# ValerioSpagnoli/Monocular-Visual-Inertial-MSCKF

Measured on AMD Instinct MI355X. Metric: MSCKF measurement-updates/sec (N=30 clones, 2000 features, track=10), higher is better.
Workload: dtype f64; 1 GPU; N=30 clones, F=2000 features, track=10, fp64; unit_definition=one 2000-feature measurement update (K1-K7)

## Files before the change

monocular-visual-inertial-msckf_amd/csrc/k_feature.h:

```cpp
#pragma once
#include <hip/hip_runtime.h>
#include "wave_ops.h"
#include "feature_dpp_groups.h"
#include "batch_order.h"

namespace msckf {


struct FeatureArgs {
    int F;
    int f0;
    int ldp;
    const int* view_ptr;
    const double* obs_uv;
    const int* obs_slot;
    const double* obs_w;
    const double* idp_base;
    const double* idp_m;
    const double* idp_rho;
    const double* cam_R;
    const double* cam_t;
    const double* cam_R0;
    const double* cam_t0;
    const double* P;
    const double* chi2;
    int n_chi2;
    double g[3];
    double Kinv[9];
    double sigma2;
    const long long* blk_off;
    void* stack;
    int stack_f32;
    int* rank;
    unsigned char* accepted;
    const unsigned char* select;
    double* gamma;
    long long* stamps;
    long long zero_idx;
    const SplitRec* split;
    int* rank_h;
    unsigned char* acc_h;
};

__host__ __device__ inline int feature_chunk_views(int M) {
    const int a = (6 * M + 63) / 64, b = (M + 9) / 10;
    const int nch = a > b ? a : b;
    return (M + nch - 1) / nch;
}
__host__ __device__ inline int feature_lds_doubles(int M, bool chunked) {
    const int R2 = 2 * M, C6 = 6 * M;
    const int head = (M + 2) / 2 + R2 * 6 + R2 * 3 + 3 * C6;
    if (!chunked) {
        const int stage = R2 * (6 * feature_chunk_views(M) + 1), elim = (R2 + 1) * (R2 + 3);
        return head + (stage > elim ? stage : elim) + 3 * R2 + 8;
    }
    const int stage = R2 * (6 * feature_chunk_views(M) + 1) + (R2 + 2), elim = (R2 + 1) * (R2 + 3);
    return head + (stage > elim ? stage : elim) + 8;
}

__host__ __device__ inline int feature_split_estride(int M) {
    const int R2 = 2 * M;
    const int cv = feature_chunk_views(M), ld = 6 * (cv > SPLIT_GSLOTS ? cv : SPLIT_GSLOTS) + 1;
    const int stage = R2 * ld, elim = (R2 + 1) * (R2 + 3);
    return (stage > elim ? stage : elim) + 8;
}
__host__ __device__ inline int feature_split_lds_doubles(int M, int nwv = 1) {
    const int R2 = 2 * M, C6 = 6 * M;
    const int head = (M + 2) / 2 + R2 * 6 + R2 * 3 + 3 * C6;
    const int cv = feature_chunk_views(M), ld = 6 * (cv > SPLIT_GSLOTS ? cv : SPLIT_GSLOTS) + 1;
    const int tail = (R2 + 2) + 8 + 6 * R2 + 6 * C6 + (M + 3 * SPLIT_MAXG + 4) / 2 + 2;
    if (nwv > 1) return head + nwv * feature_split_estride(M) + tail;
    return head + R2 * ld + tail;
}

// ... 57 lines not shown
                 : "+v"(d[0]), "+v"(d[1]), "+v"(d[2]), "+v"(d[3]) : "v"(a[0]), "v"(a[1]), "v"(a[2]), "v"(a[3]), [w] "v"(w), [lk] "i"(LK));
}
#undef MSCKF_FD
template <int LK, int J0, int NJ>
__device__ __forceinline__ void elim_from16(double (&d)[16], const double (&a)[16], double w) {
    if constexpr (NJ > 0) {
        constexpr int N1 = NJ < 4 ? NJ : 4;
        double dd[N1], aa[N1];
#pragma unroll
        for (int i = 0; i < N1; ++i) { dd[i] = d[J0 + i]; aa[i] = a[J0 + i]; }
        elim_from<LK>(dd, aa, w);
#pragma unroll
        for (int i = 0; i < N1; ++i) d[J0 + i] = dd[i];
        elim_from16<LK, J0 + N1, NJ - N1>(d, a, w);
    }
}
template <int LK, int J0, int NJ>
__device__ __forceinline__ void elim_self16(double (&d)[16], double w) {
    if constexpr (NJ > 0) {
        constexpr int N1 = NJ < 4 ? NJ : 4;
        double dd[N1];
#pragma unroll
        for (int i = 0; i < N1; ++i) dd[i] = d[J0 + i];
        elim_self<LK>(dd, w);
#pragma unroll
        for (int i = 0; i < N1; ++i) d[J0 + i] = dd[i];
        elim_self16<LK, J0 + N1, NJ - N1>(d, w);
    }
}
template <int K, int KEND, typename Fn>
__device__ __forceinline__ void feature_static_for(Fn&& fn) {
    if constexpr (K < KEND) { fn(FTag<K>{}); feature_static_for<K + 1, KEND>(fn); }
}
template <int RMAX, bool SPLIT = false, int NWV = 1>
__global__ __launch_bounds__(64 * NWV, NWV > 1 ? 1 : (RMAX <= 24 ? 3 : 2)) void k_feature(FeatureArgs p) {
    constexpr bool CHUNKED = RMAX > 32;
    static_assert(!SPLIT || CHUNKED, "the split form is an instance of the chunked kernel");
    static_assert(NWV == 1 || SPLIT, "several wavefronts per track: the split form only");
    constexpr bool ONE_CHUNK = RMAX <= 24;
    constexpr int MAXVK = ONE_CHUNK ? 10 : (RMAX - 2) / 2;
    extern __shared__ __attribute__((aligned(16))) double smem[];
    const int f = blockIdx.x + p.f0;
    const int lane = threadIdx.x & 63, wv = NWV > 1 ? (int)(threadIdx.x >> 6) : 0;
    const bool wfirst = wv == 0;
    auto xsync = [&]() { if constexpr (NWV > 1) __syncthreads(); else wave_sync(); };
    const int v0 = p.view_ptr[f];
    const int M = p.view_ptr[f + 1] - v0;
    const int R2 = 2 * M, C6 = 6 * M;
    int* sSlot = reinterpret_cast<int*>(smem);
    double* sA = smem + (M + 2) / 2;
    double* sV = sA + R2 * 6;
    double* sZ = sV + R2 * 3;

    if (f == 0 && lane < 8 && wfirst) {
        if (p.stack_f32) static_cast<float*>(p.stack)[p.zero_idx + lane] = 0.0f;
        else static_cast<double*>(p.stack)[p.zero_idx + lane] = 0.0;
    }
    auto wsum = [&](double x) -> double {
        if constexpr (RMAX <= 34) {
            x = row16_sum(x);
            return readlane_d(x, 0) + readlane_d(x, 16);
        } else {
            return wave_sum(x);
        }
    };
    if (p.select && !(p.select[f] & 1)) {
        if (lane == 0 && wfirst) {
            p.rank[f] = 0; p.gamma[f] = 0.0; p.accepted[f] = 3;
            if (p.acc_h) { p.rank_h[f] = 0; p.acc_h[f] = 3; }
            if constexpr (SPLIT) {
                const SplitRec& sr = p.split[blockIdx.x];
                for (int g = 0; g < sr.ng; ++g) if (sr.child[g] >= 0) { p.rank[sr.child[g]] = 3; p.accepted[sr.child[g]] = 3; }
                p.rank[sr.wide] = 0; p.accepted[sr.wide] = 3;
            }
        }
        return;
    }
    long long tq[8] = {0, 0, 0, 0, 0, 0, 0, 0};
    if (p.stamps) tq[0] = wall_clock64();
    double res = 0.0, a0 = 0, a1 = 0, a2 = 0, a3 = 0, a4 = 0, a5 = 0, h0 = 0, h1 = 0, h2 = 0;
    const int view = lane >> 1;
    if (lane < R2) {
        const int o = v0 + view;
        const int s = p.obs_slot[o];
        if ((lane & 1) == 0 && wfirst) sSlot[view] = s;
        const double* R = p.cam_R + 9 * s;
        const double* t = p.cam_t + 3 * s;
        const double* R0 = p.cam_R0 + 9 * s;
        const double* t0 = p.cam_t0 + 3 * s;
        const double rho = p.idp_rho[f];
        const double wx = rho * (p.idp_base[3 * f + 0] - t[0]) + p.idp_m[3 * f + 0];
        const double wy = rho * (p.idp_base[3 * f + 1] - t[1]) + p.idp_m[3 * f + 1];
        const double wz = rho * (p.idp_base[3 * f + 2] - t[2]) + p.idp_m[3 * f + 2];
        const double px = R[0] * wx + R[3] * wy + R[6] * wz;
        const double py = R[1] * wx + R[4] * wy + R[7] * wz;
        const double pz = R[2] * wx + R[5] * wy + R[8] * wz;
        const double Wx = R[0] * px + R[1] * py + R[2] * pz + t[0];
        const double Wy = R[3] * px + R[4] * py + R[5] * pz + t[1];
        const double Wz = R[6] * px + R[7] * py + R[8] * pz + t[2];
        const double u = p.obs_uv[2 * o], v = p.obs_uv[2 * o + 1];
        double wv = 1.0;
        if (p.obs_w) wv = p.obs_w[o];
        const double zx = p.Kinv[0] * u + p.Kinv[1] * v + p.Kinv[2];
        const double zy = p.Kinv[3] * u + p.Kinv[4] * v + p.Kinv[5];
        const double zw = p.Kinv[6] * u + p.Kinv[7] * v + p.Kinv[8];
        const double ia = 1.0 / pz;
        const double jb = -px * (ia * ia);
        const double jc = -py * (ia * ia);
        const double izw = 1.0 / zw;
        const double gx = p.g[0], gy = p.g[1], gz = p.g[2];
        const double u0 = R0[0] * gx + R0[3] * gy + R0[6] * gz;
        const double u1 = R0[1] * gx + R0[4] * gy + R0[7] * gz;
        const double u2 = R0[2] * gx + R0[5] * gy + R0[8] * gz;
        const double ex = Wx - t0[0], ey = Wy - t0[1], ez = Wz - t0[2];
        const double u3 = ey * gz - ez * gy;
        const double u4 = ez * gx - ex * gz;
        const double u5 = ex * gy - ey * gx;
        const double den = u0 * u0 + u1 * u1 + u2 * u2 + u3 * u3 + u4 * u4 + u5 * u5;
        double J0, J1, J2;
        if ((lane & 1) == 0) {
            res = zx * izw - px * ia;
            J0 = ia; J1 = 0.0; J2 = jb;
            a0 = -jb * py; a1 = -ia * pz + jb * px; a2 = ia * py;
        } else {
            res = zy * izw - py * ia;
            J0 = 0.0; J1 = ia; J2 = jc;
            a0 = ia * pz - jc * py; a1 = jc * px; a2 = -ia * px;
        }
        h0 = J0 * R[0] + J1 * R[1] + J2 * R[2];
        h1 = J0 * R[3] + J1 * R[4] + J2 * R[5];
        h2 = J0 * R[6] + J1 * R[7] + J2 * R[8];
        a3 = -h0; a4 = -h1; a5 = -h2;
        if (den > 1e-6) {
// ... 148 lines not shown
                for (int a = 0; a < 6; ++a) pb[VW % (PD + 1)][a] = prow[(size_t)a * p.ldp];
            }
        };
        fetch(FTag<0>{});
        if constexpr (PD > 1) fetch(FTag<1>{});
        if constexpr (PD > 2) fetch(FTag<2>{});
        if constexpr (PD > 3) fetch(FTag<3>{});
        static_assert(PD >= 1 && PD <= 4, "the prologue above issues PD views");
        {
            const double z0 = sZ[c], z1 = sZ[C6 + c], z2 = sZ[2 * C6 + c];
            const double d0 = sA[(2 * vwc) * 6 + ac], d1 = sA[(2 * vwc + 1) * 6 + ac];
            auto rows = [&](auto tagl) {
                constexpr int L0 = decltype(tagl)::value;
                if (L0 < R2) {
                    double x[4] = {0.0, 0.0, 0.0, 0.0};
                    corr(tagl, x, z0, z1, z2);
#pragma unroll
                    for (int i = 0; i < 4; ++i)
                        if (L0 + i < R2 && cok) sE[(L0 + i) * ldE + lc] = x[i];
                }
            };
            rows(FTag<0>{}); rows(FTag<4>{}); rows(FTag<8>{}); rows(FTag<12>{}); rows(FTag<16>{}); rows(FTag<20>{});
            rows(FTag<24>{}); rows(FTag<28>{});
            if (cok) {
                sE[(2 * vwc) * ldE + lc] += d0;
                sE[(2 * vwc + 1) * ldE + lc] += d1;
            }
            if (last && lane < R2) sE[lane * ldE + cw] = ro;
            wave_sync();
            const int nel = q * cwp;
            if (cw == C6) {
                const double* srcrows = sE + rank * ldE;
                if (p.stack_f32) {
                    float* blk = static_cast<float*>(p.stack) + p.blk_off[f];
                    for (int e = lane; e < nel; e += 64) blk[e] = (float)srcrows[e];
                } else {
                    double* blk = static_cast<double*>(p.stack) + p.blk_off[f];
                    int e = lane;
                    for (; e + 192 < nel; e += 256) {
                        const double x0 = srcrows[e], x1 = srcrows[e + 64], x2 = srcrows[e + 128], x3 = srcrows[e + 192];
                        blk[e] = x0; blk[e + 64] = x1; blk[e + 128] = x2; blk[e + 192] = x3;
                    }
                    for (; e < nel; e += 64) blk[e] = srcrows[e];
                }
            } else {
                const float inv_cwp = 1.0f / (float)cwp;
                for (int e = lane; e < nel; e += 64) {
                    const int L = (int)(((float)e + 0.5f) * inv_cwp), cc = e - L * cwp;
                    const double x = sE[(rank + L) * ldE + cc];
                    const long long dst = p.blk_off[f] + (long long)L * ldb + c0 + cc;
                    if (p.stack_f32) static_cast<float*>(p.stack)[dst] = (float)x;
                    else static_cast<double*>(p.stack)[dst] = x;
                }
            }
            wave_sync();
        }
        if (p.stamps && vc0 == 0) tq[3] = wall_clock64();
        {
            double zp0 = 0, zp1 = 0, zp2 = 0;
            auto view = [&](auto tagv) {
                constexpr int VW = decltype(tagv)::value;
                if (VW < M) {
                    fetch(FTag<VW + PD>{});
                    double e0 = 0.0, e1 = 0.0;
                    if constexpr (VW < MAXVK) FeatGateView<VW>::run(zp0, zp1, zp2, e0, e1, pb[VW % (PD + 1)], zq, aq);
                    if (cok) { sE[(2 * VW) * ldE + lc] = e0; sE[(2 * VW + 1) * ldE + lc] = e1; }
                }
            };
            view(FTag<0>{}); view(FTag<1>{}); view(FTag<2>{}); view(FTag<3>{}); view(FTag<4>{}); view(FTag<5>{});
            view(FTag<6>{}); view(FTag<7>{}); view(FTag<8>{}); view(FTag<9>{}); view(FTag<10>{});
            view(FTag<11>{}); view(FTag<12>{}); view(FTag<13>{}); view(FTag<14>{});
            auto rows = [&](auto tagl) {
                constexpr int L0 = decltype(tagl)::value;
                if (L0 < R2) {
                    double x[4];
#pragma unroll
                    for (int i = 0; i < 4; ++i) x[i] = sE[min(L0 + i, R2 - 1) * ldE + lc];
                    corr(tagl, x, zp0, zp1, zp2);
#pragma unroll
                    for (int i = 0; i < 4; ++i)
                        if (L0 + i < R2 && cok) sE[(L0 + i) * ldE + lc] = x[i];
                }
            };
// ... 657 lines not shown
```

monocular-visual-inertial-msckf_amd/csrc/msckf_abi.hip:

```cpp
#include <hip/hip_runtime.h>
#include <dlfcn.h>
#include <rccl/rccl.h>

#include <algorithm>
#include <atomic>
#include <chrono>
#include <condition_variable>
#include <functional>
#include <mutex>
#include <thread>
#include <unordered_map>
#include <unordered_set>
#include <pthread.h>
#include <sched.h>
#include <cmath>
#include <cstdio>
#include <cstdlib>
#include <cstring>
#include <string>
#include <vector>

#include "../../include/msckf_mi355x.h"
#include "k_feature.h"
#include "k_fold.h"
// ... 295 lines not shown
    std::vector<double> x_key;
    int x_nrec = 0;
    bool x_plan_valid = false;
    std::vector<SweepNode> x_snodes;
    std::vector<SweepFold> x_sfolds;
    int x_n_merges = 0;
    size_t x_root_off = 0, x_zero_off = 0;
    long long x_rec_base = 0;
    size_t rbuf_doubles = 0;
    size_t gather_off = 0;
    int gather_cap = 0;
    int n_leaves = 0;
    int n_leaves0 = 0;
    float us_host_prep = 0, us_h2d = 0, us_d2h = 0;
    float us_stage[3] = {0, 0, 0};
    float us_total = 0;
    std::vector<int> h_view_in;
    bool have_tracks = false, use_select = false;
    msckf_select_params sel_params{};
    std::vector<double> h_cam[4];
    bool have_nominal = false;
    Buf dNom;
    Buf dPoseArena, dFeatArena, dRawArena, dResArena, dGateArena;
    void *hPose = nullptr, *hFeat = nullptr, *hRes = nullptr, *hGate = nullptr, *hP = nullptr;
    size_t hFeatCap = 0, hGateCap = 0, res_dx_off = 0, res_p_off = 0;
    size_t res_mask_off = 0, res_mask_cap = 0, res_cap = 0;
    std::vector<int> x_bounds;
    int xmask_doubles = 0;
    Buf dPerm;
    bool have_w = false;
    size_t w_raw_off = 0;
    Buf dObsW;
    const GatherRec* gather_rec = nullptr;
    std::vector<double> chi2_cache;
    bool defer_state_sync = false;
    bool oneshot = false;
    bool feature_launched = false;
    HostPool* pool = nullptr;
    Buf dGsEx, dGsFlag, dGsProg;
    Buf dRootFlush, dXRootFlush;
    RootTables plan_tabs, merge_tabs;
    unsigned gs_epoch = 0;
    bool gs_enabled = true;
    bool gs_overlap = true;
    int root_band = 0;
    bool gs_stamp = false;
    Buf dSplit, dRem;
    static constexpr int REM_DIRECT_DEFAULT = 3840;
    int rem_leaf_rows = 0;
    int rem_direct_max = REM_DIRECT_DEFAULT, rem_direct_max_wide = 16 * GS_MAX_NB2;
    bool retry_plain = false;
    bool fake_timeout_done = false;
    bool rem_direct = false;
    std::vector<FoldNode> rnodes;
    std::vector<std::pair<int, int>> rlevels;
    int rroot = -1; size_t rroot_off = 0;
    std::vector<int> rtops;
    int rtop_rows = 0;
    int rem_cut_rows = -1;
    Buf dRNodes;
    hipEvent_t ev_rem = nullptr;
    bool wide_active = false;
    bool no_wide = false;
    hipStream_t stream2 = nullptr;
    hipEvent_t ev_fork = nullptr, ev_wfeat = nullptr;
    bool wide_on_stream2 = false;
// ... 769 lines not shown
    if (c->xchg_planned)
        HIPCHK(c, hipMemcpyAsync(c->dRbuf.p, c->h_xflags.data(), c->h_xflags.size() * 8, hipMemcpyHostToDevice, ps));
    HIPCHK(c, hipEventRecord(c->ev_plan_up[img], ps));
    c->plan_staged[img] = true;
    return MSCKF_OK;
}

inline bool rem_in_record(const msckf_ctx* c) { return c->xchg_planned && c->xsplit_rows > 0; }
inline double* rem_rows(msckf_ctx* c) { return rem_in_record(c) ? ptr<double>(c->dRbuf) + rec_rem_off(c) + 1 : ptr<double>(c->dRem); }
inline int* drem_count(msckf_ctx* c) { return reinterpret_cast<int*>(ptr<double>(c->dRem) + (size_t)16 * GS_MAX_NB2 * (6 * c->maxN + 1)); }
inline int* rem_count(msckf_ctx* c) { return rem_in_record(c) ? reinterpret_cast<int*>(ptr<double>(c->dRbuf) + rec_rem_off(c)) : drem_count(c); }

int launch_feature(msckf_ctx* c) {
    if (c->F == 0) return MSCKF_OK;
    FeatureArgs a{};
    a.F = c->F; a.ldp = c->d;
    a.view_ptr = ptr<int>(c->dViewPtr); a.obs_uv = ptr<double>(c->dObsUV); a.obs_slot = ptr<int>(c->dObsSlot);
    a.idp_base = ptr<double>(c->dBase); a.idp_m = ptr<double>(c->dMvec); a.idp_rho = ptr<double>(c->dRho);
    a.obs_w = c->have_w ? ptr<double>(c->dObsW) : nullptr;
    a.cam_R = ptr<double>(c->dCamR); a.cam_t = ptr<double>(c->dCamT);
    a.cam_R0 = ptr<double>(c->dCamR0); a.cam_t0 = ptr<double>(c->dCamT0);
    a.P = ptr<double>(c->dP); a.chi2 = ptr<double>(c->dChi2); a.n_chi2 = c->n_chi2;
    for (int i = 0; i < 3; ++i) a.g[i] = c->g[i];
    for (int i = 0; i < 9; ++i) a.Kinv[i] = c->Kinv[i];
    a.sigma2 = c->sigma * c->sigma;
    a.blk_off = ptr<long long>(c->dBlkOff); a.stack = c->dStack.p; a.stack_f32 = c->cfg.dtype == MSCKF_DTYPE_F32 ? 1 : 0;
    a.rank = ptr<int>(c->dRank); a.accepted = ptr<unsigned char>(c->dAcc); a.gamma = ptr<double>(c->dGamma);
    a.select = c->use_select ? ptr<unsigned char>(c->dSelFlags) : nullptr;
    a.stamps = c->dStamps.p ? ptr<long long>(c->dStamps) + 8 * 8192 : nullptr;
    a.zero_idx = c->ord.stack_elems;
    c->gate_direct = c->want_direct && !c->use_select;
    if (c->gate_direct) { a.rank_h = static_cast<int*>(c->hGate); a.acc_h = static_cast<unsigned char*>(c->hGate) + (size_t)c->ord.Fs * 4; }
    hipStream_t st = c->stream;
    auto go = [&](int f0, int nf, int mmax) {
        if (nf <= 0) return;
        a.f0 = f0; a.F = nf; a.split = nullptr;
        const bool chunked = 2 * mmax + 1 > 32;
        int lds_d = 0;
        for (int m = 1; m <= mmax; ++m) lds_d = std::max(lds_d, feature_lds_doubles(m, chunked));
        const size_t lds = (size_t)lds_d * 8;
        if (mmax <= 10) hipLaunchKernelGGL(k_feature<24>, dim3(nf), dim3(64), lds, st, a);
        else if (2 * mmax + 1 <= 32) hipLaunchKernelGGL(k_feature<32>, dim3(nf), dim3(64), lds, st, a);
        else hipLaunchKernelGGL(k_feature<64>, dim3(nf), dim3(64), lds, st, a);
    };
    auto go_split = [&](int f0, int nf, int mmax) {
        if (nf <= 0) return;
        a.f0 = f0; a.F = nf; a.split = ptr<SplitRec>(c->dSplit);
        static const int mw_max = [] { const char* e = std::getenv("MSCKF_SPLIT_MW_MAX"); return e ? std::atoi(e) : 512; }();
        const int nwv = nf <= mw_max ? 4 : 1;
        int lds_d = 0;
        for (int m = 2; m <= mmax; ++m) lds_d = std::max(lds_d, feature_split_lds_doubles(m, nwv));
        if (nwv == 4) hipLaunchKernelGGL((k_feature<64, true, 4>), dim3(nf), dim3(256), (size_t)lds_d * 8, st, a);
        else hipLaunchKernelGGL((k_feature<64, true>), dim3(nf), dim3(64), (size_t)lds_d * 8, st, a);
        if (c->rem_direct) {
            RemScatterArgs r{};
            r.split = ptr<SplitRec>(c->dSplit); r.n_tracks = nf; r.rows_cap = c->ord.rem_cap;
            r.dc = c->dc; r.N = c->N;
            r.view_ptr = a.view_ptr; r.obs_slot = a.obs_slot; r.blk_off = a.blk_off; r.stack = a.stack; r.stack_f32 = a.stack_f32;
            r.rank = a.rank; r.accepted = a.accepted; r.out = rem_rows(c); r.nrows = rem_count(c);
            hipLaunchKernelGGL(k_rem_scatter, dim3(nf + 1), dim3(256), 0, st, r);
        }
    };
    c->wide_on_stream2 = false;
    if (c->ord.split_on && c->ord.Fw > 0) {
        if (c->wide_concurrent) {
            HIPCHK(c, hipEventRecord(c->ev_fork, c->stream));
            HIPCHK(c, hipStreamWaitEvent(c->stream2, c->ev_fork, 0));
            st = c->stream2;
            go_split(c->ord.Fb, c->ord.Fw, c->ord.Mmax_wide);
            HIPCHK(c, hipEventRecord(c->ev_wfeat, c->stream2));
            c->wide_on_stream2 = true;
            st = c->stream;
            go(0, c->ord.Fb, c->ord.Mmax_band);
        } else {
// ... 653 lines not shown
    c->maxN = cfg->max_clones; c->maxF = cfg->max_features; c->maxM = std::min<int>(cfg->max_track, MSCKF_MAX_TRACK); c->maxV = cfg->max_track;
    if (hipSetDevice(c->device) != hipSuccess) { delete c; return MSCKF_ERR_NO_DEVICE; }
    hipDeviceProp_t prop{};
    if (hipGetDeviceProperties(&prop, c->device) != hipSuccess) { delete c; return MSCKF_ERR_NO_DEVICE; }
    if (std::strncmp(prop.gcnArchName, "gfx950", 6) != 0) { delete c; return MSCKF_ERR_NO_DEVICE; }
    c->n_cu = prop.multiProcessorCount;
    if (hipStreamCreateWithFlags(&c->stream, hipStreamNonBlocking) != hipSuccess) { delete c; return MSCKF_ERR_HIP; }
    if (hipStreamCreateWithFlags(&c->stream2, hipStreamNonBlocking) != hipSuccess) { msckf_destroy(c); return MSCKF_ERR_HIP; }
    if (hipStreamCreateWithFlags(&c->stream_up, hipStreamNonBlocking) != hipSuccess) { msckf_destroy(c); return MSCKF_ERR_HIP; }
    {
        const char* e1 = std::getenv("MSCKF_GAIN_STREAM");
        const char* e2 = std::getenv("MSCKF_GAIN_OVERLAP");
        c->gs_enabled = !(e1 && std::atoi(e1) == 0);
        { const char* e3 = std::getenv("MSCKF_WIDE_STREAM"); c->wide_concurrent = !(e3 && std::atoi(e3) == 0); }
        c->gs_overlap = !(e2 && std::atoi(e2) == 0);
        { const char* e4 = std::getenv("MSCKF_REM_LEAF_ROWS"); if (e4 && std::atoi(e4) >= 16) c->rem_leaf_rows = std::atoi(e4); }
        { const char* e5 = std::getenv("MSCKF_REM_CUT_ROWS"); if (e5 && std::atoi(e5) >= 0) c->rem_cut_rows = std::atoi(e5); }
    }
    hipError_t cerr = hipSuccess;
    const char* cwhat = "";
    auto CK = [&](hipError_t e, const char* what) { if (cerr == hipSuccess && e != hipSuccess) { cerr = e; cwhat = what; } };
    for (auto& e : c->ev) CK(hipEventCreate(&e), "hipEventCreate");
    CK(hipEventCreateWithFlags(&c->ev_fork, hipEventDisableTiming), "hipEventCreate");
    CK(hipEventCreateWithFlags(&c->ev_wfeat, hipEventDisableTiming), "hipEventCreate");
    CK(hipEventCreateWithFlags(&c->ev_rem, hipEventDisableTiming), "hipEventCreate");
    for (auto& e : c->ev_plan_up) CK(hipEventCreateWithFlags(&e, hipEventDisableTiming), "hipEventCreate");
    CK(hipEventCreateWithFlags(&c->ev_state, hipEventDisableTiming), "hipEventCreate");
    CK(hipEventCreateWithFlags(&c->ev_gate, hipEventDisableTiming), "hipEventCreate");
    if (const char* e = std::getenv("MSCKF_DIRECT_RESULT")) c->direct_enabled = std::atoi(e) != 0;
    if (const char* e = std::getenv("MSCKF_ROOT_STREAM")) c->stream_enabled = std::atoi(e) != 0;
    if (const char* e = std::getenv("MSCKF_LEAF_STREAM")) c->leaf_stream_enabled = std::atoi(e) != 0;
    if (const char* e = std::getenv("MSCKF_DEBUG_POISON")) c->ws_poison = std::atoi(e) != 0;
    if (const char* e = std::getenv("MSCKF_PLAN_MEMO")) c->plan_memo = std::atoi(e) != 0;
    auto lds_attr = [&](const void* f, int bytes, const char* what) {
        CK(hipFuncSetAttribute(f, hipFuncAttributeMaxDynamicSharedMemorySize, bytes), what);
    };
    {
#define FK(RPT, CPT) reinterpret_cast<const void*>(&k_fold<FOLD_T, FOLD_RL, RPT, CPT>)
        const void* fk[] = {FK(FOLD_RPT_LEAF, FOLD_CPT1), FK(FOLD_RPT_BIG, FOLD_CPT1), FK(FOLD_RPT_LEAF, FOLD_CPT2),
                            FK(FOLD_RPT_BIG, FOLD_CPT2), FK(FOLD_RPT_W3, FOLD_CPT3)};
#undef FK
        for (const void* f : fk) lds_attr(f, FOLD_LDS_BYTES, "k_fold LDS attribute");
    }
    lds_attr(reinterpret_cast<const void*>(&k_fold_g<FOLDG_T, 12, 6>), FOLD_LDS_BYTES, "k_fold_g LDS attribute");
    lds_attr(reinterpret_cast<const void*>(&k_fold_g<FOLDG_T, 6, 10>), FOLD_LDS_BYTES, "k_fold_g LDS attribute");
    lds_attr(reinterpret_cast<const void*>(&k_fold_g<FOLDG_T, 2, 21>), FOLD_LDS_BYTES, "k_fold_g LDS attribute");
    lds_attr(reinterpret_cast<const void*>(&k_fold_g<FOLDG_T, 1, 42>), FOLD_LDS_BYTES, "k_fold_g LDS attribute");
    {
#define SK(NR, UN) reinterpret_cast<const void*>(&k_solve_lds<NR, SOLVE_WAVES, SOLVE_ROWS, UN>)
        const void* sk[] = {SK(1, true), SK(2, true), SK(3, true), SK(1, false), SK(2, false), SK(3, false)};
#undef SK
        for (const void* f : sk) lds_attr(f, LDS_MAX_BYTES - 1024, "k_solve_lds LDS attribute");
#define SM(NR, MD) reinterpret_cast<const void*>(&k_solve_lds<NR, SOLVE_WAVES, 1, true, MD>)
        const void* sm[] = {SM(1, 1), SM(2, 1), SM(3, 1), SM(1, 2), SM(2, 2), SM(3, 2), SM(1, 3), SM(2, 3), SM(3, 3)};
#undef SM
        for (const void* f : sm) lds_attr(f, LDS_MAX_BYTES - 1024, "k_solve_lds (one-sided) LDS attribute");
    }
    lds_attr(reinterpret_cast<const void*>(&k_sweep<SWEEP_NW, SWEEP_WPF>), FOLD_LDS_BYTES, "k_sweep LDS attribute");
    lds_attr(reinterpret_cast<const void*>(&k_sweep<SWEEP_NW_BIG, 1>), FOLD_LDS_BYTES, "k_sweep<12> LDS attribute");
    lds_attr(reinterpret_cast<const void*>(&k_root_gain<SWEEP_NW, 2>), LDS_MAX_BYTES - 1024, "k_root_gain LDS attribute");
    lds_attr(reinterpret_cast<const void*>(&k_root_gain_m<SWEEP_NW, SWEEP_NW_MID, 2>), LDS_MAX_BYTES - 1024, "k_root_gain_m LDS attribute");
    lds_attr(reinterpret_cast<const void*>(&k_leaf_root_gain<SWEEP_NW, 2>), LDS_MAX_BYTES - 1024, "k_leaf_root_gain LDS attribute");
    lds_attr(reinterpret_cast<const void*>(&k_root_gain_w<SWEEP_NW, 4, 2>), LDS_MAX_BYTES - 1024, "k_root_gain_w LDS attribute");
    lds_attr(reinterpret_cast<const void*>(&k_root_gain_w<SWEEP_NW, 4, 3>), LDS_MAX_BYTES - 1024, "k_root_gain_w LDS attribute");
    lds_attr(reinterpret_cast<const void*>(&k_root_gain_w<SWEEP_NW, 6, 2>), LDS_MAX_BYTES - 1024, "k_root_gain_w LDS attribute");
    lds_attr(reinterpret_cast<const void*>(&k_root_gain_w<SWEEP_NW, 6, 3>), LDS_MAX_BYTES - 1024, "k_root_gain_w LDS attribute");
    lds_attr(reinterpret_cast<const void*>(&k_feature<64, true, 4>), LDS_MAX_BYTES - 1024, "k_feature<64, true, 4> LDS attribute");
    lds_attr(reinterpret_cast<const void*>(&k_gain_stream<1>), LDS_MAX_BYTES - 1024, "k_gain_stream<1> LDS attribute");
    lds_attr(reinterpret_cast<const void*>(&k_gain_stream<2>), LDS_MAX_BYTES - 1024, "k_gain_stream<2> LDS attribute");
    lds_attr(reinterpret_cast<const void*>(&k_gain_dense), LDS_MAX_BYTES - 1024, "k_gain_dense LDS attribute");
    lds_attr(reinterpret_cast<const void*>(&k_lsweep<8, 4, LS_RS4, true>), FOLD_LDS_BYTES, "k_lsweep<8,4> LDS attribute");
    lds_attr(reinterpret_cast<const void*>(&k_lsweep<12, 4, LS_RS4, false>), FOLD_LDS_BYTES, "k_lsweep<12,4> LDS attribute");
    lds_attr(reinterpret_cast<const void*>(&k_lsweep<SWEEP_NW, 6, LS_RS6>), FOLD_LDS_BYTES, "k_lsweep<6> LDS attribute");
    lds_attr(reinterpret_cast<const void*>(&k_lsweep<12, 6, LS_RS6, false>), FOLD_LDS_BYTES, "k_lsweep<12,6> LDS attribute");
    lds_attr(reinterpret_cast<const void*>(&k_lsweep<8, 6, LS_RS6T>), FOLD_LDS_BYTES, "k_lsweep<8,6,tall> LDS attribute");
    lds_attr(reinterpret_cast<const void*>(&k_wsweep<SWEEP_NW, 4>), FOLD_LDS_BYTES, "k_wsweep<4> LDS attribute");
    lds_attr(reinterpret_cast<const void*>(&k_wsweep<SWEEP_NW, 6>), FOLD_LDS_BYTES, "k_wsweep<6> LDS attribute");
    lds_attr(reinterpret_cast<const void*>(&k_chol<512>), LDS_MAX_BYTES - 1024, "k_chol LDS attribute");
    lds_attr(reinterpret_cast<const void*>(&k_feature<24>), LDS_MAX_BYTES - 1024, "k_feature LDS attribute");
    lds_attr(reinterpret_cast<const void*>(&k_feature<32>), LDS_MAX_BYTES - 1024, "k_feature LDS attribute");
    lds_attr(reinterpret_cast<const void*>(&k_feature<64>), LDS_MAX_BYTES - 1024, "k_feature LDS attribute");
    if (((size_t)15 * (15 + 6 * c->maxN) + 225) * 8 > (size_t)(LDS_MAX_BYTES - 1024)) { msckf_destroy(c); return MSCKF_ERR_ARG; }
    lds_attr(reinterpret_cast<const void*>(&k_propagate), LDS_MAX_BYTES - 1024, "k_propagate LDS attribute");
    if (cerr != hipSuccess) {
        std::fprintf(stderr, "msckf_create: %s: %s\n", cwhat, hipGetErrorString(cerr));
        msckf_destroy(c);
        return MSCKF_ERR_HIP;
    }
    const int N = c->maxN, d = 15 + 6 * N, dc = 6 * N;
    int rc = MSCKF_OK;
    auto E = [&](Buf& b, size_t bytes, bool z = false) { if (rc == MSCKF_OK) rc = ensure(c, b, bytes, z); };
    E(c->dP, (size_t)d * d * 8);
    E(c->dPoseArena, (size_t)24 * N * 8);
    c->res_mask_cap = ((size_t)std::max(c->maxF, 1) + 7) & ~(size_t)7;
    c->res_cap = 64 + (size_t)d * 8 + (size_t)d * d * 8 + c->res_mask_cap;
    E(c->dResArena, c->res_cap, true);
    E(c->dGateArena, (size_t)5 * std::max(c->maxF, 1));
    if (rc == MSCKF_OK) {
        set_view(c->dCamR, c->dPoseArena.p, 0, (size_t)N * 72);
        set_view(c->dCamT, c->dPoseArena.p, (size_t)9 * N * 8, (size_t)N * 24);
        set_view(c->dCamR0, c->dPoseArena.p, (size_t)12 * N * 8, (size_t)N * 72);
        set_view(c->dCamT0, c->dPoseArena.p, (size_t)21 * N * 8, (size_t)N * 24);
        c->d = 15;
        seat_result_views(c);
        bool ok = hipHostMalloc(&c->hPose, (size_t)24 * N * 8) == hipSuccess &&
                  hipHostMalloc(&c->hRes, c->res_cap) == hipSuccess &&
                  hipHostMalloc(&c->hGate, (c->hGateCap = (size_t)5 * std::max(c->maxF, 1))) == hipSuccess &&
                  hipHostMalloc(&c->hP, (size_t)d * d * 8) == hipSuccess;
        if (!ok) rc = MSCKF_ERR_HIP;
    }
    E(c->dChi2, 1024 * 8);
    E(c->dKeep, (size_t)d * 4);
    E(c->dY, (size_t)d * dc * 8); E(c->dS, (size_t)dc * dc * 8); E(c->dL, (size_t)dc * dc * 8);
// ... 124 lines not shown
    tracks_clear(c);
    return MSCKF_OK;
}

static int launch_gather_w(msckf_ctx* c) {
    const int Fs = c->ord.Fs;
    char* draw = static_cast<char*>(c->dRawArena.p);
    HIPCHK(c, hipMemcpyAsync(draw + c->w_raw_off, static_cast<char*>(c->hFeat) + c->w_raw_off, (size_t)c->sumM * 8, hipMemcpyHostToDevice, c->stream));
    hipLaunchKernelGGL(k_gather_w, dim3((Fs + GATHER_THREADS / 32 - 1) / (GATHER_THREADS / 32)), dim3(GATHER_THREADS), 0, c->stream,
                       c->gather_rec, reinterpret_cast<const double*>(draw + c->w_raw_off), ptr<double>(c->dObsW), Fs, c->sumM, c->ord.sumMs);
    HIPCHK(c, hipGetLastError());
    return MSCKF_OK;
}

static int set_features_impl(msckf_ctx* c, int32_t F, const int32_t* view_ptr, const double* obs_uv,
                             const int32_t* obs_slot, const double* idp_base, const double* idp_m,
                             const double* idp_rho, const TrackEmitSrc* emit, const double* sigma_view = nullptr) {
    if (!c || F < 0 || F > c->maxF) return MSCKF_ERR_ARG;
    if (!c->have_state) return MSCKF_ERR_STATE;
    if (F > 0 && (!view_ptr || !obs_slot || (!emit && (!obs_uv || !idp_base || !idp_m || !idp_rho)))) return MSCKF_ERR_ARG;
    HIPCHK(c, hipSetDevice(c->device));
    const double t0 = now_us();
    const int N = c->N;
    if (c->feat_busy) { HIPCHK(c, hipStreamSynchronize(c->stream)); c->feat_busy = false; }
    c->have_features = false;
    c->feature_launched = false;
    c->last.ran = false;
    c->have_tracks = false;
    c->use_select = false;
    c->batch_from_store = false;
    c->no_wide = false;
    c->have_w = false;
    c->gather_rec = nullptr;
    if (F == 0) {
        c->F = 0;
        c->sumM = 0; c->ord.reset(); c->nodes.clear(); c->levels.clear(); c->snodes.clear(); c->sfolds.clear(); c->sweep_levels.clear(); c->n_group_merges = 0;
        c->band_plan = false; c->root = -1;
        c->wide_active = false;
        c->rem_direct = false;
        c->rnodes.clear(); c->rlevels.clear(); c->rroot = -1; c->rtops.clear(); c->rtop_rows = 0;
        c->plan_valid = false;
        c->xchg_planned = false;
        if (c->xchg) {
            const size_t need = (rec_head(c) + (size_t)N * rec_slot(c) + rec_rem_doubles(c) + 16) * 8;
            if (int rcw = workspace_room(c, need, need, c->stream)) return rcw;
            c->ws_key_valid = false;
            HIPCHK(c, hipMemsetAsync(c->dRbuf.p, 0, rec_head(c) * 8, c->stream));
            if (c->xsplit_rows > 0) HIPCHK(c, hipMemsetAsync(ptr<double>(c->dRbuf) + rec_rem_off(c), 0, 8, c->stream));
            HIPCHK(c, hipStreamSynchronize(c->stream));
            c->xchg_planned = true;
            c->rbuf_doubles = rec_head(c) + (size_t)N * rec_slot(c) + rec_rem_doubles(c);
            c->gather_off = c->rbuf_doubles;
        }
        c->have_features = true;
        c->us_host_prep = (float)(now_us() - t0);
        return MSCKF_OK;
    }
    if (view_ptr[0] != 0) return MSCKF_ERR_ARG;
    for (int f = 0; f < F; ++f) {
        const int M = view_ptr[f + 1] - view_ptr[f];
        if (M < 1 || M > c->maxM) return MSCKF_ERR_ARG;
    }
    const int sumM = view_ptr[F];
    const RawLayout raw = raw_layout(F, sumM);
    const size_t w_off = (raw.pin_bytes + 15) & ~(size_t)15, img_bytes = w_off + (size_t)sumM * 8;
    if (c->hFeatCap < img_bytes) {
// ... 98 lines not shown
    set_view(c->dObsW, c->dFeatArena.p, so_w_off, (size_t)sumMs * 8);
    if ((size_t)5 * Fs > c->dGateArena.bytes || (size_t)5 * Fs > c->hGateCap) {
        HIPCHK(c, hipStreamSynchronize(c->stream));
        if (int rcg = ensure(c, c->dGateArena, (size_t)8 * Fs)) return rcg;
        if (c->hGate) HIPCHK(c, hipHostFree(c->hGate));
        c->hGate = nullptr; c->hGateCap = 0;
        HIPCHK(c, hipHostMalloc(&c->hGate, (size_t)8 * Fs));
        c->hGateCap = (size_t)8 * Fs;
    }
    set_view(c->dRank, c->dGateArena.p, 0, (size_t)Fs * 4);
    set_view(c->dAcc, c->dGateArena.p, (size_t)Fs * 4, (size_t)Fs);
    int rc = MSCKF_OK;
    auto E = [&](Buf& b, size_t bytes, bool z = false) { if (rc == MSCKF_OK) rc = ensure(c, b, bytes, z); };
    const size_t stack_es = c->cfg.dtype == MSCKF_DTYPE_F32 ? 4 : 8;
    E(c->dStack, ((size_t)ord.stack_elems + 8) * stack_es); E(c->dGamma, (size_t)F * 8);
    if (ord.split_on) E(c->dSplit, ord.h_split.size() * sizeof(SplitRec));
    if (rc != MSCKF_OK) { (void)hipStreamSynchronize(c->stream); return rc; }
    if (!zc) HIPCHK(c, hipMemcpyAsync(draw + raw.raw_bytes, hb + raw.raw_bytes, (size_t)Fs * sizeof(GatherRec), hipMemcpyHostToDevice, c->stream));
    if (ord.split_on) HIPCHK(c, hipMemcpyAsync(c->dSplit.p, hb + split_off, ord.h_split.size() * sizeof(SplitRec), hipMemcpyHostToDevice, c->stream));
    if (c->oneshot) HIPCHK(c, hipEventRecord(c->ev[6], c->stream));
    if (emit) {
        if (int rce = launch_track_emit(c, emit, F, sumM, view_ptr, draw, raw)) return rce;
    }
    {
        GatherArgs g;
        g.uv_in = reinterpret_cast<const double*>(draw);
        g.slot_in = reinterpret_cast<const int*>(draw + raw.r_slot); g.base_in = reinterpret_cast<const double*>(draw + raw.r_base);
        g.m_in = reinterpret_cast<const double*>(draw + raw.r_m); g.rho_in = reinterpret_cast<const double*>(draw + raw.r_rho);
        g.rec = reinterpret_cast<const GatherRec*>((zc ? hb : draw) + raw.raw_bytes);
        g.uv = ptr<double>(c->dObsUV); g.base = ptr<double>(c->dBase); g.m = ptr<double>(c->dMvec); g.rho = ptr<double>(c->dRho);
        g.slot = ptr<int>(c->dObsSlot); g.fmin = ptr<int>(c->dFmin); g.view = ptr<int>(c->dViewPtr); g.perm = ptr<int>(c->dPerm);
        g.blk = ptr<long long>(c->dBlkOff); g.info = ptr<FeatInfo>(c->dFeatInfo);
        g.F = Fs; g.sumM = sumMs;
        hipLaunchKernelGGL(k_gather, dim3((Fs + GATHER_THREADS / 32 - 1) / (GATHER_THREADS / 32)), dim3(GATHER_THREADS), 0, c->stream, g);
        HIPCHK(c, hipGetLastError());
        c->gather_rec = g.rec;
    }
    if (sigma_view) {
        if (int rcw = launch_gather_w(c)) return rcw;
        c->have_w = true;
    }
    c->feature_launched = false;
    if (c->state_pending) { HIPCHK(c, hipStreamWaitEvent(c->stream, c->ev_state, 0)); c->state_pending = false; }
    c->gate_event = false;
    if (c->oneshot) {
        if (int rcf = launch_feature(c)) return rcf;
        c->feature_launched = true;
        if (c->gate_direct) { HIPCHK(c, hipEventRecord(c->ev_gate, c->stream)); c->gate_event = true; }
    }
    const double t2 = now_us();
    const bool plan_hit = c->plan_valid && !c->plan_no_wide && c->plan_N == N && c->plan_xchg == c->xchg && c->plan_view == h_view &&
                          c->plan_fmin == h_fmin && c->plan_fmax == h_fmax;
    if (!plan_hit) {
        c->plan_valid = false;
        plan_batch(c, h_fmin, h_fmax, h_view);
        c->plan_N = N; c->plan_xchg = c->xchg; c->plan_view = h_view;
    }
    c->gather_off = c->rbuf_doubles;
    const double t3 = now_us();
    c->us_host_prep = (float)((t1 - t0) + (t3 - t2));
    if (!plan_hit) {
        const size_t need = (c->rbuf_doubles + 16) * 8;
        const bool side = c->oneshot || !c->run_pending;
        c->plan_stream = side ? c->stream_up : c->stream;
        if (int rcw = workspace_room(c, need, need + need / 2, c->plan_stream)) { c->plan_stream = nullptr; return rcw; }
        const bool keep = c->ws_head && c->ws_key_valid && c->ws_key_p == c->dRbuf.p && c->ws_key_dc == c->dc;
        if (!keep) HIPCHK(c, hipMemsetAsync(c->dRbuf.p, 0, need, c->plan_stream));
        else if (c->ws_poison) {
// ... 1863 lines not shown
```

Before: 3404 updates/s.

## Fuse the gather kernel into the feature kernel on the one-shot path

When the one-shot path runs without emit or splitting and tracks are short, the feature kernel now reads each track's gather record itself. It loads the raw observations and feature parameters directly and still writes the gathered arrays (uv, slot, base, fmin, info, view, perm, blk) for later stages. This removes the separate k_gather launch and one round trip of the observation data through global memory. In exchange, the feature kernel gains extra prologue work and wave syncs, and it always uses the 24 or 32 instantiation.

```diff
diff --git a/monocular-visual-inertial-msckf_amd/csrc/k_feature.h b/monocular-visual-inertial-msckf_amd/csrc/k_feature.h
--- a/monocular-visual-inertial-msckf_amd/csrc/k_feature.h
+++ b/monocular-visual-inertial-msckf_amd/csrc/k_feature.h
@@ -3,6 +3,7 @@
 #include "wave_ops.h"
 #include "feature_dpp_groups.h"
 #include "batch_order.h"
+#include "k_gather.h"
 
 namespace msckf {
 
@@ -40,6 +41,7 @@
     const SplitRec* split;
     int* rank_h;
     unsigned char* acc_h;
+    GatherArgs gather;
 };
 
 __host__ __device__ inline int feature_chunk_views(int M) {
@@ -163,11 +165,12 @@
 __device__ __forceinline__ void feature_static_for(Fn&& fn) {
     if constexpr (K < KEND) { fn(FTag<K>{}); feature_static_for<K + 1, KEND>(fn); }
 }
-template <int RMAX, bool SPLIT = false, int NWV = 1>
+template <int RMAX, bool SPLIT = false, int NWV = 1, bool GATHER = false>
 __global__ __launch_bounds__(64 * NWV, NWV > 1 ? 1 : (RMAX <= 24 ? 3 : 2)) void k_feature(FeatureArgs p) {
     constexpr bool CHUNKED = RMAX > 32;
     static_assert(!SPLIT || CHUNKED, "the split form is an instance of the chunked kernel");
     static_assert(NWV == 1 || SPLIT, "several wavefronts per track: the split form only");
+    static_assert(!GATHER || (!CHUNKED && NWV == 1), "the gathered form: k_feature<24> and <32>");
     constexpr bool ONE_CHUNK = RMAX <= 24;
     constexpr int MAXVK = ONE_CHUNK ? 10 : (RMAX - 2) / 2;
     extern __shared__ __attribute__((aligned(16))) double smem[];
@@ -175,8 +178,21 @@
     const int lane = threadIdx.x & 63, wv = NWV > 1 ? (int)(threadIdx.x >> 6) : 0;
     const bool wfirst = wv == 0;
     auto xsync = [&]() { if constexpr (NWV > 1) __syncthreads(); else wave_sync(); };
-    const int v0 = p.view_ptr[f];
-    const int M = p.view_ptr[f + 1] - v0;
+    int v0, M;
+    int cf = f, ain = 0;
+    long long boff = 0;
+    if constexpr (GATHER) {
+        long long w = 0;
+        if (lane < 3) w = reinterpret_cast<const long long*>(p.gather.rec + f)[lane];
+        const int wl = (int)w, wh = (int)(w >> 32);
+        cf = __builtin_amdgcn_readlane(wl, 0); ain = __builtin_amdgcn_readlane(wh, 0);
+        M = __builtin_amdgcn_readlane(wl, 1); v0 = __builtin_amdgcn_readlane(wh, 1);
+        boff = ((long long)__builtin_amdgcn_readlane(wh, 2) << 32) | (unsigned)__builtin_amdgcn_readlane(wl, 2);
+    } else {
+        v0 = p.view_ptr[f];
+        M = p.view_ptr[f + 1] - v0;
+    }
+    auto blk_off_f = [&]() -> long long { if constexpr (GATHER) return boff; else return p.blk_off[f]; };
     const int R2 = 2 * M, C6 = 6 * M;
     int* sSlot = reinterpret_cast<int*>(smem);
     double* sA = smem + (M + 2) / 2;
@@ -195,6 +211,51 @@
             return wave_sum(x);
         }
     };
+    int g_slot = 0;
+    double g_u = 0.0, g_v = 0.0;
+    if constexpr (GATHER) {
+        const GatherArgs& g = p.gather;
+        const int gview = lane >> 1;
+        const bool grow = lane < 2 * M;
+        int sl = 1 << 30;
+        double hv = 0.0;
+        if (grow) {
+            sl = g.slot_in[ain + gview];
+            const double2 q = *reinterpret_cast<const double2*>(g.uv_in + 2 * (size_t)(ain + gview));
+            g_u = q.x; g_v = q.y;
+        }
+        if (lane < 3) hv = g.base_in[3 * (size_t)cf + lane];
+        else if (lane < 6) hv = g.m_in[3 * (size_t)cf + lane - 3];
+        else if (lane == 6) hv = g.rho_in[cf];
+        if (grow && (lane & 1) == 0) {
+            *reinterpret_cast<double2*>(g.uv + 2 * (size_t)(v0 + gview)) = make_double2(g_u, g_v);
+            g.slot[v0 + gview] = sl;
+        }
+        int lo = sl;
+#pragma unroll
+        for (int k = 32; k >= 1; k >>= 1) lo = min(lo, __shfl_xor(lo, k, 64));
+        unsigned long long* scol = reinterpret_cast<unsigned long long*>(sA);
+        if (lane < 2) scol[lane] = ~0ull;
+        wave_sync();
+        if (grow && (lane & 1) == 0 && sl - lo < 16) reinterpret_cast<unsigned char*>(scol)[sl - lo] = (unsigned char)gview;
+        wave_sync();
+        if (lane < 3) g.base[3 * (size_t)f + lane] = hv;
+        else if (lane < 6) g.m[3 * (size_t)f + lane - 3] = hv;
+        else if (lane == 6) g.rho[f] = hv;
+        else if (lane == 7) g.fmin[f] = lo;
+        else if (lane == 8) {
+            FeatInfo fi;
+            fi.blk_off = boff; fi.M = M; fi.pad = 0;
+            *reinterpret_cast<unsigned long long*>(fi.col) = scol[0];
+            *reinterpret_cast<unsigned long long*>(fi.col + 8) = scol[1];
+            g.info[f] = fi;
+        } else if (lane == 9) {
+            g.view[f] = v0; g.perm[f] = cf; g.blk[f] = boff;
+            if (f == g.F - 1) g.view[g.F] = g.sumM;
+        }
+        wave_sync();
+        g_slot = sl;
+    }
     if (p.select && !(p.select[f] & 1)) {
         if (lane == 0 && wfirst) {
             p.rank[f] = 0; p.gamma[f] = 0.0; p.accepted[f] = 3;
@@ -213,23 +274,25 @@
     const int view = lane >> 1;
     if (lane < R2) {
         const int o = v0 + view;
-        const int s = p.obs_slot[o];
+        const int s = GATHER ? g_slot : p.obs_slot[o];
         if ((lane & 1) == 0 && wfirst) sSlot[view] = s;
         const double* R = p.cam_R + 9 * s;
         const double* t = p.cam_t + 3 * s;
         const double* R0 = p.cam_R0 + 9 * s;
         const double* t0 = p.cam_t0 + 3 * s;
-        const double rho = p.idp_rho[f];
-        const double wx = rho * (p.idp_base[3 * f + 0] - t[0]) + p.idp_m[3 * f + 0];
-        const double wy = rho * (p.idp_base[3 * f + 1] - t[1]) + p.idp_m[3 * f + 1];
-        const double wz = rho * (p.idp_base[3 * f + 2] - t[2]) + p.idp_m[3 * f + 2];
+        const double* ibase = GATHER ? p.gather.base_in + 3 * (size_t)cf : p.idp_base + 3 * f;
+        const double* im = GATHER ? p.gather.m_in + 3 * (size_t)cf : p.idp_m + 3 * f;
+        const double rho = GATHER ? p.gather.rho_in[cf] : p.idp_rho[f];
+        const double wx = rho * (ibase[0] - t[0]) + im[0];
+        const double wy = rho * (ibase[1] - t[1]) + im[1];
+        const double wz = rho * (ibase[2] - t[2]) + im[2];
         const double px = R[0] * wx + R[3] * wy + R[6] * wz;
         const double py = R[1] * wx + R[4] * wy + R[7] * wz;
         const double pz = R[2] * wx + R[5] * wy + R[8] * wz;
         const double Wx = R[0] * px + R[1] * py + R[2] * pz + t[0];
         const double Wy = R[3] * px + R[4] * py + R[5] * pz + t[1];
         const double Wz = R[6] * px + R[7] * py + R[8] * pz + t[2];
-        const double u = p.obs_uv[2 * o], v = p.obs_uv[2 * o + 1];
+        const double u = GATHER ? g_u : p.obs_uv[2 * o], v = GATHER ? g_v : p.obs_uv[2 * o + 1];
         double wv = 1.0;
         if (p.obs_w) wv = p.obs_w[o];
         const double zx = p.Kinv[0] * u + p.Kinv[1] * v + p.Kinv[2];
@@ -444,10 +507,10 @@
             if (cw == C6) {
                 const double* srcrows = sE + rank * ldE;
                 if (p.stack_f32) {
-                    float* blk = static_cast<float*>(p.stack) + p.blk_off[f];
+                    float* blk = static_cast<float*>(p.stack) + blk_off_f();
                     for (int e = lane; e < nel; e += 64) blk[e] = (float)srcrows[e];
                 } else {
-                    double* blk = static_cast<double*>(p.stack) + p.blk_off[f];
+                    double* blk = static_cast<double*>(p.stack) + blk_off_f();
                     int e = lane;
                     for (; e + 192 < nel; e += 256) {
                         const double x0 = srcrows[e], x1 = srcrows[e + 64], x2 = srcrows[e + 128], x3 = srcrows[e + 192];
@@ -460,7 +523,7 @@
                 for (int e = lane; e < nel; e += 64) {
                     const int L = (int)(((float)e + 0.5f) * inv_cwp), cc = e - L * cwp;
                     const double x = sE[(rank + L) * ldE + cc];
-                    const long long dst = p.blk_off[f] + (long long)L * ldb + c0 + cc;
+                    const long long dst = blk_off_f() + (long long)L * ldb + c0 + cc;
                     if (p.stack_f32) static_cast<float*>(p.stack)[dst] = (float)x;
                     else static_cast<double*>(p.stack)[dst] = x;
                 }
diff --git a/monocular-visual-inertial-msckf_amd/csrc/msckf_abi.hip b/monocular-visual-inertial-msckf_amd/csrc/msckf_abi.hip
--- a/monocular-visual-inertial-msckf_amd/csrc/msckf_abi.hip
+++ b/monocular-visual-inertial-msckf_amd/csrc/msckf_abi.hip
@@ -351,6 +351,9 @@
     size_t w_raw_off = 0;
     Buf dObsW;
     const GatherRec* gather_rec = nullptr;
+    bool gather_enabled = true;
+    bool feat_gather = false;
+    GatherArgs gather_args{};
     std::vector<double> chi2_cache;
     bool defer_state_sync = false;
     bool oneshot = false;
@@ -1186,6 +1189,9 @@
     c->gate_direct = c->want_direct && !c->use_select;
     if (c->gate_direct) { a.rank_h = static_cast<int*>(c->hGate); a.acc_h = static_cast<unsigned char*>(c->hGate) + (size_t)c->ord.Fs * 4; }
     hipStream_t st = c->stream;
+    const bool gather = c->feat_gather;
+    c->feat_gather = false;
+    if (gather) a.gather = c->gather_args;
     auto go = [&](int f0, int nf, int mmax) {
         if (nf <= 0) return;
         a.f0 = f0; a.F = nf; a.split = nullptr;
@@ -1193,7 +1199,10 @@
         int lds_d = 0;
         for (int m = 1; m <= mmax; ++m) lds_d = std::max(lds_d, feature_lds_doubles(m, chunked));
         const size_t lds = (size_t)lds_d * 8;
-        if (mmax <= 10) hipLaunchKernelGGL(k_feature<24>, dim3(nf), dim3(64), lds, st, a);
+        if (gather) {
+            if (mmax <= 10) hipLaunchKernelGGL((k_feature<24, false, 1, true>), dim3(nf), dim3(64), lds, st, a);
+            else hipLaunchKernelGGL((k_feature<32, false, 1, true>), dim3(nf), dim3(64), lds, st, a);
+        } else if (mmax <= 10) hipLaunchKernelGGL(k_feature<24>, dim3(nf), dim3(64), lds, st, a);
         else if (2 * mmax + 1 <= 32) hipLaunchKernelGGL(k_feature<32>, dim3(nf), dim3(64), lds, st, a);
         else hipLaunchKernelGGL(k_feature<64>, dim3(nf), dim3(64), lds, st, a);
     };
@@ -1913,6 +1922,7 @@
     if (const char* e = std::getenv("MSCKF_LEAF_STREAM")) c->leaf_stream_enabled = std::atoi(e) != 0;
     if (const char* e = std::getenv("MSCKF_DEBUG_POISON")) c->ws_poison = std::atoi(e) != 0;
     if (const char* e = std::getenv("MSCKF_PLAN_MEMO")) c->plan_memo = std::atoi(e) != 0;
+    if (const char* e = std::getenv("MSCKF_FEATURE_GATHER")) c->gather_enabled = std::atoi(e) != 0;
     auto lds_attr = [&](const void* f, int bytes, const char* what) {
         CK(hipFuncSetAttribute(f, hipFuncAttributeMaxDynamicSharedMemorySize, bytes), what);
     };
@@ -1960,6 +1970,8 @@
     lds_attr(reinterpret_cast<const void*>(&k_chol<512>), LDS_MAX_BYTES - 1024, "k_chol LDS attribute");
     lds_attr(reinterpret_cast<const void*>(&k_feature<24>), LDS_MAX_BYTES - 1024, "k_feature LDS attribute");
     lds_attr(reinterpret_cast<const void*>(&k_feature<32>), LDS_MAX_BYTES - 1024, "k_feature LDS attribute");
+    lds_attr(reinterpret_cast<const void*>(&k_feature<24, false, 1, true>), LDS_MAX_BYTES - 1024, "k_feature LDS attribute");
+    lds_attr(reinterpret_cast<const void*>(&k_feature<32, false, 1, true>), LDS_MAX_BYTES - 1024, "k_feature LDS attribute");
     lds_attr(reinterpret_cast<const void*>(&k_feature<64>), LDS_MAX_BYTES - 1024, "k_feature LDS attribute");
     if (((size_t)15 * (15 + 6 * c->maxN) + 225) * 8 > (size_t)(LDS_MAX_BYTES - 1024)) { msckf_destroy(c); return MSCKF_ERR_ARG; }
     lds_attr(reinterpret_cast<const void*>(&k_propagate), LDS_MAX_BYTES - 1024, "k_propagate LDS attribute");
@@ -2150,6 +2162,7 @@
     c->no_wide = false;
     c->have_w = false;
     c->gather_rec = nullptr;
+    c->feat_gather = false;
     if (F == 0) {
         c->F = 0;
         c->sumM = 0; c->ord.reset(); c->nodes.clear(); c->levels.clear(); c->snodes.clear(); c->sfolds.clear(); c->sweep_levels.clear(); c->n_group_merges = 0;
@@ -2314,8 +2327,19 @@
         g.slot = ptr<int>(c->dObsSlot); g.fmin = ptr<int>(c->dFmin); g.view = ptr<int>(c->dViewPtr); g.perm = ptr<int>(c->dPerm);
         g.blk = ptr<long long>(c->dBlkOff); g.info = ptr<FeatInfo>(c->dFeatInfo);
         g.F = Fs; g.sumM = sumMs;
-        hipLaunchKernelGGL(k_gather, dim3((Fs + GATHER_THREADS / 32 - 1) / (GATHER_THREADS / 32)), dim3(GATHER_THREADS), 0, c->stream, g);
-        HIPCHK(c, hipGetLastError());
+        const bool fuse = c->gather_enabled && c->oneshot && !emit && !ord.split_on && Fs == F && 2 * ord.Mmax + 1 <= 32;
+        if (fuse) {
+            if (c->ws_poison) {
+                HIPCHK(c, hipMemsetAsync(c->dFeatArena.p, 0xFF, so_w_off, c->stream));
+                if (c->dFeatArena.bytes > so_bytes)
+                    HIPCHK(c, hipMemsetAsync(static_cast<char*>(c->dFeatArena.p) + so_bytes, 0xFF, c->dFeatArena.bytes - so_bytes, c->stream));
+            }
+            c->gather_args = g;
+            c->feat_gather = true;
+        } else {
+            hipLaunchKernelGGL(k_gather, dim3((Fs + GATHER_THREADS / 32 - 1) / (GATHER_THREADS / 32)), dim3(GATHER_THREADS), 0, c->stream, g);
+            HIPCHK(c, hipGetLastError());
+        }
         c->gather_rec = g.rec;
     }
     if (sigma_view) {
```

New measurement: 3158 updates/s. 7.2% lower.
